# althonos/pyrodigal

Hardware: AMD Instinct MI355X
Metric: Mbp/sec gene-called (meta mode) (higher is better)
Workload: dtype f64; 1 GPU; 100000x20kbp_gc30-70_meta; contigs=100000, bases=2000000000, models=16, contigs_rank0=100000, sub_batch_contigs=6250, contexts_per_gpu=4, genes_all_ranks=2908995, steps_issued=a join of the contexts and a gather per step

## Files before the change

### pyrodigal_amd/csrc/finder.hip

```cpp
#include "pga_internal.h"
#include "pipeline.h"
#include "dpw_core.h"
#include "dev_common.h"
#include "find_plan.h"

#include <math.h>
#include <stdio.h>
#include <stdlib.h>
#include <string.h>

#include <algorithm>
#include <atomic>
#include <chrono>
#include <condition_variable>
#include <functional>
#include <limits>
#include <map>
#include <memory>
#include <mutex>
#include <new>
#include <thread>
#include <type_traits>
#include <unordered_map>

// ... 1004 lines not shown
    HT(c, hipMalloc((void**)&f->d_model_gc, sizeof(double) * nm));
    HT(c, hipMalloc((void**)&f->d_model_grp, sizeof(int32_t) * nm));
    HT(c, hipMemcpy(f->d_model_gc, mgc.data(), sizeof(double) * nm, hipMemcpyHostToDevice));
    HT(c, hipMemcpy(f->d_model_grp, f->model_group.data(), sizeof(int32_t) * nm, hipMemcpyHostToDevice));
    {
        const int ng = (int)f->group_tt.size();
        std::vector<int32_t> rank(nm, 0), count(ng, 0);
        for (int m = 0; m < nm; m++) rank[m] = count[f->model_group[m]]++;
        size_t total_il = 0;
        for (int g = 0; g < ng; g++) { f->gil_stride.push_back((count[g] + 1) & ~1); f->gil_off.push_back(total_il); total_il += (size_t)4096 * f->gil_stride[g]; }
        std::vector<double> il(total_il + 8, 0.0);
        for (int m = 0; m < nm; m++) {
            const int g = f->model_group[m];
            for (int h = 0; h < 4096; h++) il[f->gil_off[g] + (size_t)h * f->gil_stride[g] + rank[m]] = c->models[m].gene_dc[h];
        }
        HT(c, hipMalloc((void**)&f->d_gil, sizeof(double) * il.size()));
        HT(c, hipMalloc((void**)&f->d_model_rank, sizeof(int32_t) * nm));
        HT(c, hipMemcpy(f->d_gil, il.data(), sizeof(double) * il.size(), hipMemcpyHostToDevice));
        HT(c, hipMemcpy(f->d_model_rank, rank.data(), sizeof(int32_t) * nm, hipMemcpyHostToDevice));
        f->model_rank = rank;
    }
    return PGA_OK;
}

struct pga_batch {
    pga_ctx* ctx;
    int32_t n;
    int64_t total;
    std::vector<ContigDesc> ct;
    char* d_seq;
    size_t d_seq_cap = 0;
    TileDesc* d_tiles;
    int32_t* d_tile0;
    int32_t n_tiles;
    int mask_case = 0;
    std::vector<int32_t> reg_off;
    std::vector<MaskRun> regions;
    MaskRun* d_regions = nullptr;
    std::vector<uint8_t> circular;
    std::vector<int32_t> sets;
};

static void batch_tiles(const pga_batch* b, std::vector<TileDesc>& tiles, std::vector<int32_t>& tile0) {
    const int TS = pga_extract_tile_size();
    tile0.resize((size_t)b->n + 1);
    for (int i = 0; i < b->n; i++) {
        tile0[i] = (int32_t)tiles.size();
        const int64_t L = b->ct[i].len;
        if (L >= 3) for (int64_t s0 = 0; s0 < L; s0 += TS) tiles.push_back(TileDesc{i, (int32_t)s0});
    }
    tile0[b->n] = (int32_t)tiles.size();
}
static size_t batch_tiles_bytes(const std::vector<TileDesc>& tiles, const std::vector<int32_t>& tile0) {
    return sizeof(TileDesc) * tiles.size() + sizeof(int32_t) * tile0.size() + 64 + 256;
}
static hipError_t batch_upload_tiles(pga_batch* b, char* at, const std::vector<TileDesc>& tiles, const std::vector<int32_t>& tile0, hipStream_t st) {
    b->n_tiles = (int32_t)tiles.size();
    const size_t tb = sizeof(TileDesc) * tiles.size(), zb = sizeof(int32_t) * tile0.size();
    b->d_tiles = (TileDesc*)(((uintptr_t)at + 255) & ~(uintptr_t)255);
    b->d_tile0 = (int32_t*)((char*)b->d_tiles + tb);
    hipError_t e = hipSuccess;
    if (tb) e = hipMemcpyAsync(b->d_tiles, tiles.data(), tb, hipMemcpyHostToDevice, st);
    if (e == hipSuccess) e = hipMemcpyAsync(b->d_tile0, tile0.data(), zb, hipMemcpyHostToDevice, st);
    return e;
}

extern "C" int pga_dp_start_order(int32_t n_chains, const int32_t* nodes_per_chain, int32_t* order) {
    if (n_chains < 0 || (n_chains > 0 && (!nodes_per_chain || !order))) return PGA_EINVAL;
    int maxb = 0;
    for (int k = 0; k < n_chains; k++) maxb = std::max(maxb, std::max(nodes_per_chain[k], 0) >> 6);
    std::vector<int32_t> first((size_t)maxb + 2, 0);
    for (int k = 0; k < n_chains; k++) first[(size_t)(maxb - (std::max(nodes_per_chain[k], 0) >> 6)) + 1]++;
    for (int b = 0; b <= maxb; b++) first[(size_t)b + 1] += first[(size_t)b];
    for (int k = 0; k < n_chains; k++) order[(size_t)first[(size_t)(maxb - (std::max(nodes_per_chain[k], 0) >> 6))]++] = k;
    return PGA_OK;
}

extern "C" int64_t pga_dp_xcd_order(int32_t n_chains, const int32_t* order, const int32_t* nodes_per_chain, const int32_t* key_of_chain, int32_t n_keys,
                                    int32_t* out, int64_t out_cap) {
    if (n_chains < 0 || n_keys < 0 || (n_chains > 0 && (!order || !nodes_per_chain || !key_of_chain || !out))) return -(int64_t)PGA_EINVAL;
    std::vector<int32_t> queue[8];
    int64_t load[8] = {0, 0, 0, 0, 0, 0, 0, 0};
    std::vector<int8_t> xcd_of((size_t)n_keys, (int8_t)-1);
    for (int p = 0; p < n_chains; p++) {
        const int c = order[p];
        if (c < 0 || c >= n_chains || key_of_chain[c] < 0 || key_of_chain[c] >= n_keys) return -(int64_t)PGA_EINVAL;
        int8_t& x = xcd_of[(size_t)key_of_chain[c]];
        if (x < 0) { int best = 0; for (int q = 1; q < 8; q++) if (load[q] < load[best]) best = q; x = (int8_t)best; }
        queue[x].push_back(c);
        load[x] += std::max(nodes_per_chain[c], 0);
    }
    size_t longest = 0;
    for (int q = 0; q < 8; q++) longest = std::max(longest, queue[q].size());
// ... 420 lines not shown
    if (kn.fault_contig_len_set) {
        const long fl = kn.fault_contig_len;
        for (int i = 0; i < NC; i++) if ((long)batch->ct[i].len == fl) { c->err = "pga_find_genes: fault injected by PGA_FAULT_CONTIG_LEN"; return PGA_EDEVICE; }
    }
    if (use_sets) {
        NS = pga_plan::dense_set_ids(batch->sets.data(), NC, set_of);
        c->set_model.assign((size_t)NC, -1);
        c->set_score.assign((size_t)NC, std::numeric_limits<double>::quiet_NaN());
        c->model_scores.assign((size_t)NC * (size_t)NM, std::numeric_limits<double>::quiet_NaN());
        c->model_scores_nm = NM;
    }
    R = new (std::nothrow) ResultOwner();
    if (!R) return PGA_ENOMEM;
    R->contigs.assign(NC, pga_contig_result{-1, 0, 0, 0, 0, 0.0, 0.0});
    R->mask_off.assign(NC + 1, 0);
    R->has_masks = P.mask || mask_union;
    memset(&R->pub, 0, sizeof R->pub);
    R->pub.n_contigs = NC;
    total = batch->total;
    return PGA_OK;
}

int FindCall::run_sequence_and_masks() {
    const char* d_seq = batch->d_seq;
    DEVSET(d_dig, uint8_t, "d_dig", total + 16);
    DEVSET(d_ct, ContigDesc, "d_ct", NC + 1);
    const size_t xa_cnt = 4, xa_cbase = xa_cnt + 2 * (size_t)NC, xa_sbase = xa_cbase + (size_t)NG * (NC + 1), xa_en = xa_sbase + (size_t)NG * (NC + 1);
    xa_words = xa_en + ((size_t)NG * NC + 3) / 4 + 1;
    DEVSET(d_xa, int32_t, "d_extract_info", xa_words);
    PINSET(h_xa, int32_t, "h_extract_info", xa_words);
    d_cnt = d_xa + xa_cnt; h_cnt = h_xa + xa_cnt;
    const int64_t gc_blocks = pga_gc_blocks(total);
    DEVSET(d_p16, int32_t, "d_gc_p16", total / 16 + 2);
    DEVBUF(d_gc_bsum, int32_t, "d_gc_bsum", gc_blocks + 1);
    DEVBUF(d_gc_boff, int32_t, "d_gc_boff", gc_blocks + 1);
    d_cbase = d_xa + xa_cbase; h_cbase = h_xa + xa_cbase;
    DEVSET(d_tile_first, int32_t, "d_tile_first", (size_t)6 * batch->n_tiles);
    DEVSET(d_tile_last, int32_t, "d_tile_last", (size_t)6 * batch->n_tiles);
    DEVSET(d_tile.count, int32_t, "d_tile_count", (size_t)NG * (batch->n_tiles + 1));
    DEVSET(d_tile.off, int32_t, "d_tile_off", (size_t)NG * (batch->n_tiles + 1));
    DEVSET(d_tile.scount, int32_t, "d_tile_scount", (size_t)NG * (batch->n_tiles + 1));
    DEVSET(d_tile.soff, int32_t, "d_tile_soff", (size_t)NG * (batch->n_tiles + 1));
    d_sbase = d_xa + xa_sbase; h_sbase = h_xa + xa_sbase;
    d_enabled = (uint8_t*)(d_xa + xa_en); h_enabled = (uint8_t*)(h_xa + xa_en);

    for (int g = 0; g < NG; g++) {
        GBUF(df, uint8_t, total + 16)
        GBUF(c16, int32_t, (size_t)batch->n_tiles * 192 + 2)
        ga[g].tile0 = batch->d_tile0;
        ga[g].ndx = nullptr; ga[g].stop_val = nullptr; ga[g].type = nullptr; ga[g].strand = nullptr; ga[g].edge0 = nullptr; ga[g].gc_cont = nullptr;
    }

    HT(c, hipEventRecord(f->e_start, st));
    HT(c, hipMemcpyAsync(d_ct, batch->ct.data(), sizeof(ContigDesc) * (NC + 1), hipMemcpyHostToDevice, st));
    HT(c, hipMemsetAsync(d_xa, 0, sizeof(int32_t) * xa_cbase, st));
    pga_launch_digitize(d_seq, d_dig, total, d_ct, NC, d_cnt, d_cnt + NC, st);
    pga_launch_gc_prefix(d_dig, total, d_gc_bsum, d_gc_boff, d_p16, st);
    if (mask_union) {
        const int64_t per_source = total / std::max(1, P.min_mask) + NC + 1;
        const int64_t most = std::min<int64_t>((P.mask ? per_source : 0) + (batch->mask_case ? per_source : 0) + (int64_t)batch->regions.size(),
                                               total / 2 + NC + 1);
        const int cap = (int)std::min<int64_t>(most, (int64_t)1 << 28);
        DEVBUF(d_bits, uint32_t, "d_mask_bits", 2 * pga_mask_words(total) + 2);
        DEVBUF(d_mcounts, int32_t, "d_mask_counts", 4 * (pga_mask_waves(total) + 1));
        DEVBUF(d_moff, int32_t, "d_mask_off", NC + 2);
        DEVBUF(d_miv, int2, "d_mask_iv", cap + 1);
        PINBUF(h_moff_, int32_t, "h_mask_off", NC + 2);
        pga_launch_mask_union(d_dig, d_seq, total, d_ct, NC, batch->d_tiles, batch->n_tiles, P.mask, batch->mask_case, P.min_mask, batch->d_regions,
                              (int)batch->regions.size(), d_bits, d_mcounts, d_moff, d_miv, cap, st);
        HT(c, hipMemcpyAsync(h_moff_, d_moff, sizeof(int32_t) * (NC + 1), hipMemcpyDeviceToHost, st));
        h_moff = h_moff_; d_union_iv = d_miv;
        masks = MaskList{d_moff, d_miv};
    } else if (P.mask) {
        const int cap = (int)std::min<int64_t>(total / std::max(1, P.min_mask) + NC + 1, (int64_t)1 << 28);
        DEVBUF(d_runs, MaskRun, "d_mask_runs", cap + 1);
        DEVBUF(d_nruns, int32_t, "d_mask_count", 4);
        DEVBUF(d_moff, int32_t, "d_mask_off", NC + 2);
        DEVBUF(d_miv, int2, "d_mask_iv", cap + 1);
        pga_launch_find_masks(d_dig, d_ct, NC, batch->d_tiles, batch->n_tiles, P.min_mask, d_runs, d_nruns, cap, st);
        int32_t nruns = 0;
        HT(c, hipMemcpyAsync(&nruns, d_nruns, 4, hipMemcpyDeviceToHost, st));
        HT(c, hipStreamSynchronize(st));
        nruns = std::min(nruns, cap);
        std::vector<MaskRun> runs((size_t)nruns);
        if (nruns > 0) HT(c, hipMemcpy(runs.data(), d_runs, sizeof(MaskRun) * nruns, hipMemcpyDeviceToHost));
        std::sort(runs.begin(), runs.end(), [](const MaskRun& a, const MaskRun& b) { return a.contig != b.contig ? a.contig < b.contig : a.begin < b.begin; });
        std::vector<int32_t> moff(NC + 1, 0);
        std::vector<int2> miv((size_t)nruns + 1);
        for (int k = 0; k < nruns; k++) { moff[runs[k].contig + 1]++; miv[k] = make_int2(runs[k].begin, runs[k].end); }
        for (int i = 0; i < NC; i++) moff[i + 1] += moff[i];
// ... 1091 lines not shown
```

### pyrodigal_amd/csrc/pipeline.h

```cpp
#pragma once
#include "pga_internal.h"

#define PGA_STAGE_SLACK 8
struct TileDesc {
    int32_t contig;
    int32_t start;
};

struct GroupArrays {
    uint8_t* df;
    int32_t* c16; const int32_t* tile0 = nullptr;
    int32_t* st_ndx; int32_t* st_sv;
    uint8_t* st_info;
    int32_t st_half = 0; int32_t* st_overflow = nullptr;
    int32_t* stop_list;
    int32_t* start_list = nullptr;
    uint32_t* ovl_topo;
    int32_t* srank = nullptr;
    int32_t* ndx; int32_t* stop_val; uint8_t* type; int8_t* strand; uint8_t* edge0; float* gc_cont;
    int32_t* contig_of = nullptr;
};

struct ChainArrays {
    double* cscore; double* sscore; double* rscore; double* uscore; double* tscore; double* mot_score;
    double* cscore_raw;
    int32_t* star_ptr;
    int32_t* mot_ndx;
    uint8_t* rbs;
    uint8_t* edge;
    uint8_t* mot_len; uint8_t* mot_spacer; uint8_t* mot_spacendx;
    double* cs_sink = nullptr;
};

struct ModelScoreConst {
    double lfac_min, lfac_max;
    double lfac_tab[1001];
};

struct MaskList {
    const int32_t* off;
    const int2* iv;
};
struct MaskRun { int32_t contig, begin, end, _pad; };

struct ScoreParams {
    int32_t closed, is_meta, max_overlap, n_models;
    double* cs_out;
    uint8_t* conv_flag;
    unsigned long long* prof = nullptr;
    int32_t models_per_pass = 512;
    int32_t lean_stops = 0;
};

void pga_launch_digitize(const char* d_seq, uint8_t* d_dig, int64_t total, const ContigDesc* d_ct, int n_contigs,
                         int32_t* d_gc, int32_t* d_unk, hipStream_t st);
int64_t pga_gc_blocks(int64_t total);
void pga_launch_gc_prefix(const uint8_t* d_dig, int64_t total, int32_t* d_block_sum, int32_t* d_block_off, int32_t* d_p16, hipStream_t st);
void pga_launch_extract(const uint8_t* d_dig, int64_t total, const ContigDesc* d_ct, int n_contigs, int tt,
                        const pga_params& p, const GroupArrays& ga, const TileDesc* d_tiles, int n_tiles, const int32_t* d_tile0,
                        int32_t* d_tile_first, int32_t* d_tile_last, int32_t* d_tile_count, int32_t* d_tile_off, int32_t* d_cbase,
                        int32_t* d_tile_scount, int32_t* d_tile_soff, int32_t* d_sbase ,
                        MaskList masks, hipStream_t st,
                        const uint8_t* d_enabled = nullptr ,
                        int ex_c = 4 ,
                        int ex_pool = 128 );
void pga_launch_place(const ContigDesc* d_ct, const TileDesc* d_tiles, int n_tiles, const int32_t* d_tile_off, const int32_t* d_tile_soff,
                      const GroupArrays& ga, hipStream_t st);
int32_t pga_mm_tiles(const ChainDesc* h_chains, int n_chains, const int32_t* h_cbase, const int32_t* h_sbase, int n_models, int tile, std::vector<int64_t>& scratch);
size_t pga_mm_scratch_bytes(int n_models, int n_chains);
constexpr size_t PGA_SS_REC_BYTES = 32, PGA_SS_MMCHAIN_BYTES = 32, PGA_SS_MMTILE_BYTES = 16;
void pga_launch_group_enable(const ContigDesc* d_ct, int n_contigs, const int32_t* d_gc_count, const double* d_model_gc,
                             const int32_t* d_model_group, int n_models, int n_groups, uint8_t* d_enabled, hipStream_t st);
void pga_launch_group_enable_sets(const ContigDesc* d_ct, int n_contigs, const int32_t* d_gc_count, const int32_t* d_set_of, int32_t* d_pool,
                                  const double* d_model_gc, const int32_t* d_model_group, int n_models, int n_groups, uint8_t* d_enabled,
                                  hipStream_t st);
void pga_launch_find_masks(const uint8_t* d_dig, const ContigDesc* d_ct, int n_contigs, const TileDesc* d_tiles, int n_tiles, int min_mask,
                           MaskRun* d_runs, int32_t* d_count, int cap, hipStream_t st);
int64_t pga_mask_words(int64_t total);
int64_t pga_mask_waves(int64_t total);
void pga_launch_mask_union(const uint8_t* d_dig, const char* d_seq, int64_t total, const ContigDesc* d_ct, int n_contigs, const TileDesc* d_tiles,
                           int n_tiles, int unknown_runs, int lower_case_runs, int min_mask, const MaskRun* d_regions, int n_regions,
                           uint32_t* d_bits, int32_t* d_counts, int32_t* d_moff, int2* d_miv, int cap, hipStream_t st);
int pga_extract_tile_size();
void pga_launch_orf_gc(const ContigDesc* d_ct, int n_contigs, const uint8_t* d_dig, const int32_t* d_p16, const GroupArrays& ga,
                       int n_nodes_total, const int32_t* d_node_contig_base, hipStream_t st);
struct ScoreGroup {
    const ChainDesc* d_chains = nullptr; int n_chains = 0; int64_t node_begin = 0, total = 0;
    const ChainDesc* d_all_chains = nullptr; const int2* d_contig_chains = nullptr;
    const int32_t* d_node_contig_base = nullptr; int n_contigs = 0; int group_nodes = 0;
    const uint8_t* d_dig = nullptr; const ContigDesc* d_ct = nullptr; const GroupArrays* ga = nullptr; const ChainArrays* ca = nullptr;
// ... 38 lines not shown
```

### pyrodigal_amd/csrc/pipeline.hip

```cpp

#include "pga_internal.h"
#include "pipeline.h"
#include <atomic>
#include "dev_common.h"
#include "dpw_core.h"

namespace {

enum { NA = 0, NG = 1, NC = 2, NT = 3, NN = 6 };

__device__ __forceinline__ int find_contig(const ContigDesc* __restrict__ ct, int n, int64_t g) {
    int lo = 0, hi = n - 1;
    while (lo < hi) { int mid = (lo + hi + 1) >> 1; if (ct[mid].base <= g) lo = mid; else hi = mid - 1; }
    return lo;
}

__device__ __forceinline__ int block_contig(const ContigDesc* __restrict__ ct, int n, int64_t block_first, int64_t g, int* s_slot) {
    int c = block_search_le([&](const int k) { return ct[k].base; }, n, block_first, s_slot);
    while (c + 1 < n && ct[c + 1].base <= g) c++;
    return c;
}
__device__ __forceinline__ int block_chain(const ChainDesc* __restrict__ ch, int n, int64_t block_first, int64_t g, int* s_slot) {
    int c = block_search_le([&](const int k) { return ch[k].off; }, n, block_first, s_slot);
    while (c + 1 < n && ch[c + 1].off <= g) c++;
    return c;
}

__device__ __forceinline__ double readlane_f64_pl(double v, int lane) {
    const int lo = __builtin_amdgcn_readlane(__double2loint(v), lane);
    const int hi = __builtin_amdgcn_readlane(__double2hiint(v), lane);
    return __hiloint2double(hi, lo);
}

__device__ __forceinline__ int sbase(const uint8_t* __restrict__ d, int L, int i, int strand) {
    return strand == 1 ? d[i] : (d[L - 1 - i] ^ 3);
}
__device__ __forceinline__ int comp2(int d) { return d <= 3 ? (d ^ 3) : NN; }
__device__ __forceinline__ int is_gc_n(int d) { return d != NA && d != NT; }

__host__ __device__ __forceinline__ bool codon_is_stop(int x0, int x1, int x2, int tt) {
    if (x0 != NT) {
        if (tt == 2) return x0 == NA && x1 == NG && (x2 == NA || x2 == NG);
        return false;
    }
    const unsigned long long taa = (1ULL<<1)|(1ULL<<2)|(1ULL<<3)|(1ULL<<4)|(1ULL<<5)|(1ULL<<9)|(1ULL<<10)|(1ULL<<11)|(1ULL<<12)|(1ULL<<13)
                                 | (1ULL<<15)|(1ULL<<16)|(1ULL<<21)|(1ULL<<22)|(1ULL<<23)|(1ULL<<24)|(1ULL<<25)|(1ULL<<26)|(1ULL<<32);
    const unsigned long long tag = (1ULL<<1)|(1ULL<<2)|(1ULL<<3)|(1ULL<<4)|(1ULL<<5)|(1ULL<<9)|(1ULL<<10)|(1ULL<<11)|(1ULL<<12)|(1ULL<<13)
                                 | (1ULL<<14)|(1ULL<<21)|(1ULL<<23)|(1ULL<<24)|(1ULL<<25)|(1ULL<<26)|(1ULL<<33);
    const unsigned long long tga = (1ULL<<1)|(1ULL<<6)|(1ULL<<11)|(1ULL<<12)|(1ULL<<15)|(1ULL<<16)|(1ULL<<22)|(1ULL<<23)|(1ULL<<26)
                                 | (1ULL<<29)|(1ULL<<30)|(1ULL<<32);
    if (x1 == NA && x2 == NG) return (tag >> tt) & 1;
    if (x1 == NG && x2 == NA) return (tga >> tt) & 1;
    if (x1 == NA && x2 == NA) return (taa >> tt) & 1;
    if (tt == 22) return x1 == NC && x2 == NA;
// ... 4 lines not shown
    if (x1 != NT || x2 != NG) return false;
    if (x0 == NA) return true;
    if (tt == 6 || tt == 10 || tt == 14 || tt == 15 || tt == 16 || tt == 2) return false;
    if (x0 == NG) return !(tt == 1 || tt == 3 || tt == 12 || tt == 2);
    if (x0 == NT) return !(tt < 4 || tt == 9 || (tt >= 21 && tt < 25));
    return false;
}
__device__ __forceinline__ bool is_stop_at(const uint8_t* __restrict__ d, int L, int i, int strand, int tt) {
    return codon_is_stop(sbase(d, L, i, strand), sbase(d, L, i + 1, strand), sbase(d, L, i + 2, strand), tt);
}

__device__ __forceinline__ int digit_of(int ch, int& gc, int& unk) {
    switch (ch) {
        case 'A': case 'a': return NA;
        case 'T': case 't': return NT;
        case 'G': case 'g': gc++; return NG;
        case 'C': case 'c': gc++; return NC;
        default: unk++; return NN;
    }
}

__device__ __forceinline__ unsigned digits4(const unsigned w, int& gc, int& unk) {
    const unsigned u = w & 0xdfdfdfdfu;
    auto eq = [](const unsigned v) {
        return (~(((v & 0x7f7f7f7fu) + 0x7f7f7f7fu) | v | 0x7f7f7f7fu)) >> 7;
    };
    const unsigned a = eq(u ^ 0x41414141u), g = eq(u ^ 0x47474747u), c = eq(u ^ 0x43434343u), t = eq(u ^ 0x54545454u);
    const unsigned n = ~(a | g | c | t) & 0x01010101u;
    gc += __popc(g | c); unk += __popc(n);
    return g | (c << 1) | t | (t << 1) | (n << 1) | (n << 2);
}

constexpr int DG_BLOCK = 16384;
__global__ void __launch_bounds__(256)
k_digitize(const char* __restrict__ seq, uint8_t* __restrict__ dig, int64_t total,
           const ContigDesc* __restrict__ ct, int n_contigs, int32_t* __restrict__ gc_count, int32_t* __restrict__ unk_count) {
    __shared__ int s_c0;
    const int64_t blk0 = (int64_t)blockIdx.x * DG_BLOCK;
    int c = block_contig(ct, n_contigs, blk0, blk0, &s_c0);
    uint4 v[4];
#pragma unroll
    for (int q = 0; q < 4; q++) {
        const int64_t g0 = blk0 + q * 4096 + (int64_t)threadIdx.x * 16;
        v[q] = g0 + 16 <= total ? *reinterpret_cast<const uint4*>(seq + g0) : make_uint4(0, 0, 0, 0);
    }
    int acc_c = -1, acc_gc = 0, acc_unk = 0;
#pragma unroll
    for (int q = 0; q < 4; q++) {
        const int64_t g0 = blk0 + q * 4096 + (int64_t)threadIdx.x * 16;
        const bool in = g0 < total;
        if (in) while (c + 1 < n_contigs && ct[c + 1].base <= g0) c++;
        int gc = 0, unk = 0;
        bool one_contig = true;
        if (in) {
            const int64_t next = ct[c + 1 <= n_contigs ? c + 1 : n_contigs].base;
            if (g0 + 16 <= total && g0 + 16 <= next) {
                const uint4 o = make_uint4(digits4(v[q].x, gc, unk), digits4(v[q].y, gc, unk), digits4(v[q].z, gc, unk), digits4(v[q].w, gc, unk));
                *reinterpret_cast<uint4*>(dig + g0) = o;
            } else {
                one_contig = false;
                int cc = c;
                for (int k = 0; k < 16 && g0 + k < total; k++) {
                    const int64_t g = g0 + k;
                    while (cc + 1 < n_contigs && ct[cc + 1].base <= g) cc++;
                    int a = 0, u = 0;
                    dig[g] = (uint8_t)digit_of(seq[g], a, u);
                    if (a) atomicAdd(&gc_count[cc], 1);
                    if (u) atomicAdd(&unk_count[cc], 1);
                }
            }
        }
        const int c0 = __builtin_amdgcn_readfirstlane(c);
        const bool uniform = __all(!in || (one_contig && c == c0));
        if (uniform) {
            int a = in ? gc : 0, u = in ? unk : 0;
#pragma unroll
            for (int m = 32; m >= 1; m >>= 1) { a += __shfl_xor(a, m, 64); u += __shfl_xor(u, m, 64); }
            if (acc_c != c0) {
                if ((threadIdx.x & 63) == 0 && acc_c >= 0) { if (acc_gc) atomicAdd(&gc_count[acc_c], acc_gc); if (acc_unk) atomicAdd(&unk_count[acc_c], acc_unk); }
                acc_c = c0; acc_gc = 0; acc_unk = 0;
            }
            acc_gc += a; acc_unk += u;
        } else if (in && one_contig) {
            if (gc) atomicAdd(&gc_count[c], gc);
            if (unk) atomicAdd(&unk_count[c], unk);
        }
    }
    __shared__ int s_c[4], s_g[4], s_u[4];
    const int wv = threadIdx.x >> 6;
    if ((threadIdx.x & 63) == 0) { s_c[wv] = acc_c; s_g[wv] = acc_gc; s_u[wv] = acc_unk; }
    __syncthreads();
    if (threadIdx.x == 0) {
#pragma unroll
        for (int w = 0; w < 4; w++) {
            if (s_c[w] < 0) continue;
            int g = s_g[w], u = s_u[w];
#pragma unroll
            for (int v = w + 1; v < 4; v++) if (s_c[v] == s_c[w]) { g += s_g[v]; u += s_u[v]; s_c[v] = -1; }
            if (g) atomicAdd(&gc_count[s_c[w]], g);
            if (u) atomicAdd(&unk_count[s_c[w]], u);
        }
    }
}

constexpr int EX_TILE = 3072;
constexpr int EX_PER_THREAD = 12;
constexpr int EX_NONE_HI = 0x7fffffff;

__device__ __forceinline__ unsigned pack4(const unsigned w, const bool comp) {
    unsigned c = w & 0x03030303u;
    if (comp) { const unsigned nm = (w >> 2) & 0x01010101u; c = (c ^ 0x03030303u) ^ (nm | (nm << 1)); }
    return (c | (c >> 6) | (c >> 12) | (c >> 18)) & 0xffu;
}
__device__ __forceinline__ unsigned long long pack16(const uint4 v, const bool comp) {
    return (unsigned long long)(pack4(v.x, comp) | (pack4(v.y, comp) << 8) | (pack4(v.z, comp) << 16) | (pack4(v.w, comp) << 24));
}
__device__ __forceinline__ unsigned long long pairrev64(unsigned long long x) {
    x = __brevll(x);
    return ((x & 0x5555555555555555ull) << 1) | ((x >> 1) & 0x5555555555555555ull);
}

struct TileGeom {
    int L, a, len;
// ... 482 lines not shown
            const int ndx = ga.st_ndx[s0 + j], info = ga.st_info[s0 + j];
            k = off + j;
            ga.ndx[k] = ndx; ga.stop_val[k] = ga.st_sv[s0 + j]; ga.type[k] = info & 3; ga.strand[k] = (info >> 3) & 1 ? -1 : 1; ga.edge0[k] = (info >> 2) & 1;
            ga.contig_of[k] = td.contig;
            const int g_hi = (ndx - td.start) >> 4, g_lo = j == 0 ? 0 : ((ga.st_ndx[s0 + j - 1] - td.start) >> 4) + 1;
            for (int g = g_lo; g <= g_hi; g++) c16[g] = k;
            if (j == cnt - 1) for (int g = g_hi + 1; g < n_groups; g++) c16[g] = off + cnt;
            is_stop = (info & 3) == PGA_T_STOP;
        }
        const unsigned long long bal = __ballot(is_stop);
        if (lane == 0) s_w[wv] = __popcll(bal);
        __syncthreads();
        const int stops_before = srun + (wv ? s_w[0] : 0) + __popcll(bal & ((1ull << lane) - 1ull));
        if (is_stop) ga.stop_list[stops_before] = k;
        else if (j < cnt && ga.start_list != nullptr) ga.start_list[start0 + j - (stops_before - tile_soff[blockIdx.x])] = k;
        srun += s_w[0] + s_w[1];
        __syncthreads();
    }
}

__device__ __forceinline__ int gcn16(const uint4 v, const int nbytes ) {
    const unsigned w[4] = {v.x, v.y, v.z, v.w};
    int n = 0;
#pragma unroll
    for (int q = 0; q < 4; q++) {
        unsigned b = (w[q] ^ (w[q] >> 1)) & 0x01010101u;
        const int keep = nbytes - 4 * q;
        if (keep <= 0) b = 0; else if (keep < 4) b &= (1u << (8 * keep)) - 1u;
        n += __popc(b);
    }
    return n;
}
__global__ void __launch_bounds__(256)
k_gcp_blocks(const uint8_t* __restrict__ dig, int64_t total, int32_t* __restrict__ block_sum) {
    __shared__ int s_w[4];
    const int64_t g0 = (int64_t)blockIdx.x * 4096 + (int64_t)threadIdx.x * 16;
    int n = 0;
    if (g0 < total) n = gcn16(*reinterpret_cast<const uint4*>(dig + g0), (int)min((int64_t)16, total - g0));
#pragma unroll
    for (int m = 32; m >= 1; m >>= 1) n += __shfl_xor(n, m, 64);
    if ((threadIdx.x & 63) == 0) s_w[threadIdx.x >> 6] = n;
    __syncthreads();
    if (threadIdx.x == 0) block_sum[blockIdx.x] = s_w[0] + s_w[1] + s_w[2] + s_w[3];
}
__global__ void __launch_bounds__(256)
k_gcp_final(const uint8_t* __restrict__ dig, int64_t total, const int32_t* __restrict__ block_off, int32_t* __restrict__ p16) {
    __shared__ int s_w[4];
    const int64_t g0 = (int64_t)blockIdx.x * 4096 + (int64_t)threadIdx.x * 16;
    int n = 0;
    if (g0 < total) n = gcn16(*reinterpret_cast<const uint4*>(dig + g0), (int)min((int64_t)16, total - g0));
    int inc = n;
    const int lane = threadIdx.x & 63, w = threadIdx.x >> 6;
#pragma unroll
    for (int off = 1; off < 64; off <<= 1) { const int v = __shfl_up(inc, off, 64); if (lane >= off) inc += v; }
    if (lane == 63) s_w[w] = inc;
    __syncthreads();
    int run = block_off[blockIdx.x] + inc - n;
    for (int k = 0; k < w; k++) run += s_w[k];
    if (g0 <= total) p16[g0 >> 4] = run;
}
__device__ __forceinline__ int gc_prefix(const uint8_t* __restrict__ dig, const int32_t* __restrict__ p16, const int64_t x) {
    const int r = (int)(x & 15);
    int n = p16[x >> 4];
    if (r) n += gcn16(*reinterpret_cast<const uint4*>(dig + (x - r)), r);
    return n;
}

__global__ void __launch_bounds__(256)
k_orf_gc(const ContigDesc* __restrict__ ct, int n_contigs, const uint8_t* __restrict__ dig, const int32_t* __restrict__ p16, GroupArrays ga,
         int n_nodes_total, const int32_t* __restrict__ node_contig_base ) {
    const int i = blockIdx.x * blockDim.x + threadIdx.x;
    if (i >= n_nodes_total) return;
    if (ga.type[i] == PGA_T_STOP) { ga.gc_cont[i] = 0.f; return; }
    const int lo = ga.contig_of[i];
    const int L = ct[lo].len;
    const int64_t base = ct[lo].base;
    auto P = [&](const int x) { return gc_prefix(dig, p16, base + x); };
    const int ndx = ga.ndx[i], sv = ga.stop_val[i];
    int cnt;
    if (ga.strand[i] == 1) {
        cnt = P(sv + 3) - P(ndx);
    } else {
        const int hi2 = min(ndx + 2, L - 1);
        cnt = (P(sv + 1) - P(sv - 2)) + (hi2 >= sv + 3 ? P(hi2 + 1) - P(sv + 3) : 0);
    }
    const double gsize = abs(sv - ndx) + 3.0;
    ga.gc_cont[i] = (float)((double)cnt / gsize);
}

__device__ __forceinline__ int hexamer(const uint8_t* __restrict__ d, int pos, int strand) {
    int v = 0;
    if (strand == 1) { for (int j = 0; j < 6; j++) v |= (d[pos + j] & 3) << (2 * j); }
    else             { for (int j = 0; j < 6; j++) v |= (comp2(d[pos - j] & 7) & 3) << (2 * j); }
    return v;
}

constexpr int CS_MODELS = 4;
constexpr int CS_LONG = 192;
constexpr int CSQ_SERIAL_MAX = 256;

struct OrfCtx {
    const uint8_t* d;
    const int32_t* c16;
    int tbase, p, q, L, strand, step, ncod;
    int kstop;
    int2 cc;
    __device__ __forceinline__ bool node_at(const int j) const { return (d[j] >> (strand == 1 ? 4 : 5)) & 1; }
    __device__ __forceinline__ int node_index(const int j) const {
        const int r = j & 15;
        uint4 v; __builtin_memcpy(&v, d + (j - r), 16);
        const unsigned w[4] = {v.x, v.y, v.z, v.w};
        int n = c16[j >> 4] - tbase;
#pragma unroll
        for (int q = 0; q < 4; q++) {
            const int keep = r - 4 * q;
            unsigned m = w[q] & 0x30303030u;
            if (keep <= 0) m = 0; else if (keep < 4) m &= (1u << (8 * keep)) - 1u;
// ... 1788 lines not shown
    const OvlChain C{ga.ndx + tb, ga.stop_val + tb, ga.type + tb, ga.strand + tb, ca.cscore + ch.off, ca.sscore + ch.off, ca.rscore + ch.off,
                     ca.uscore + ch.off, ch.n, css != nullptr ? css + ch.off : nullptr};
    overlapping_starts_ahead(C, i, my, !rev, mc, maxov, sp, K, edge0 != 1 ? neighbours : 0x80000000u, ext != nullptr ? topo_q2 + tb : nullptr);
    ca.star_ptr[3 * g] = sp[0]; ca.star_ptr[3 * g + 1] = sp[1]; ca.star_ptr[3 * g + 2] = sp[2];
    if (ext != nullptr) {
        DpwExt e;
        e.vm = 0;
#pragma unroll
        for (int k = 0; k < 3; k++) {
            e.x[k] = 0.0; e.dlo[k] = INT_MAX; e.dhi[k] = INT_MIN; e.cq[k] = DPW_NONE;
            if (sp[k] < 0) continue;
            e.vm |= 1 << k;
            e.x[k] = K.v[k];
            if (rev && e.x[k] > 0.0) {
                const int n3n = K.nd[k], n3s = K.sv[k];
                int hi = n3s + DPW_MAX_OPP_OVLP - 5;
                const int h2 = (n3n + n3s - 6) >> 1;
                if (h2 < hi) hi = h2;
                if (my - 4 < hi) hi = my - 4;
                e.dlo[k] = n3s - 5; e.dhi[k] = hi;
            }
            if (rev) e.cq[k] = K.q2[k];
        }
        ext[p] = e;
    }
}

}

static inline unsigned nblocks(int64_t n, int t) { return (unsigned)((n + t - 1) / t); }

int64_t pga_gc_blocks(int64_t total) { return (total + 1 + 4095) / 4096; }

void pga_launch_digitize(const char* d_seq, uint8_t* d_dig, int64_t total, const ContigDesc* d_ct, int n_contigs,
                         int32_t* d_gc, int32_t* d_unk, hipStream_t st) {
    if (total <= 0) return;
    hipLaunchKernelGGL(k_digitize, dim3(nblocks(total, DG_BLOCK)), dim3(256), 0, st, d_seq, d_dig, total, d_ct, n_contigs, d_gc, d_unk);
}

struct RunOfUnknown {
    static __device__ __forceinline__ bool is(const uint8_t b) { return b == NN; }
    static __device__ __forceinline__ bool all8(const uint64_t w) { return w == 0x0606060606060606ull; }
};
struct RunOfLowerCase {
    static __device__ __forceinline__ bool is(const uint8_t b) { return (unsigned)(b - 'a') < 26u; }
    static __device__ __forceinline__ bool all8(const uint64_t w) {
        const uint64_t H = 0x8080808080808080ull;
        if (w & H) return false;
        return ((w + 0x1f1f1f1f1f1f1f1full) & H) == H
            && ((w + 0x0505050505050505ull) & H) == 0;
    }
};

template <class Run, class Emit>
__device__ __forceinline__ void find_runs(const uint8_t* __restrict__ src, const ContigDesc* __restrict__ ct, const TileDesc* __restrict__ tiles,
                                          const int n_tiles, const int n_contigs, const int min_mask, Emit emit) {
    if ((int)blockIdx.x >= n_tiles) {
        const int c = ((int)blockIdx.x - n_tiles) * blockDim.x + threadIdx.x;
        if (c >= n_contigs) return;
        const ContigDesc cd = ct[c];
        if (cd.len < 1 || cd.len > 2) return;
        const uint8_t* __restrict__ d = src + cd.base;
        for (int i = 0; i < cd.len; i++) {
            if (!Run::is(d[i]) || (i > 0 && Run::is(d[i - 1]))) continue;
            int e = i + 1;
            while (e < cd.len && Run::is(d[e])) e++;
            if (e - i >= min_mask || e == cd.len) emit(c, i, e);
        }
        return;
    }
// ... 127 lines not shown
        S &= S - 1u;
        if (ks < cap) iv[ks].x = (int)(g - ct[find_contig(ct, n_contigs, g)].base);
        ks++;
    }
    while (E) {
        const int64_t g = w * 32 + __builtin_ctz(E);
        E &= E - 1u;
        if (ke < cap) iv[ke].y = (int)(g + 1 - ct[find_contig(ct, n_contigs, g)].base);
        ke++;
    }
}

int64_t pga_mask_words(int64_t total) { return (total + 32) / 32; }
int64_t pga_mask_waves(int64_t total) { return (pga_mask_words(total) + 63) / 64; }

void pga_launch_mask_union(const uint8_t* d_dig, const char* d_seq, int64_t total, const ContigDesc* d_ct, int n_contigs, const TileDesc* d_tiles,
                           int n_tiles, int unknown_runs, int lower_case_runs, int min_mask, const MaskRun* d_regions, int n_regions,
                           uint32_t* d_bits, int32_t* d_counts, int32_t* d_moff, int2* d_miv, int cap, hipStream_t st) {
    const int64_t nw = pga_mask_words(total), nwv = pga_mask_waves(total);
    uint32_t* const d_cbits = d_bits + nw;
    int32_t* const cnt_s = d_counts; int32_t* const cnt_e = cnt_s + (nwv + 1); int32_t* const off_s = cnt_e + (nwv + 1); int32_t* const off_e = off_s + (nwv + 1);
    (void)hipMemsetAsync(d_bits, 0, sizeof(uint32_t) * 2 * (size_t)nw, st);
    const dim3 run_grid(n_tiles + (n_contigs + 255) / 256);
    if (unknown_runs) hipLaunchKernelGGL(k_mask_paint_runs<RunOfUnknown>, run_grid, dim3(256), 0, st, d_dig, d_ct, d_tiles, n_tiles, n_contigs, min_mask, d_bits);
    if (lower_case_runs) hipLaunchKernelGGL(k_mask_paint_runs<RunOfLowerCase>, run_grid, dim3(256), 0, st, (const uint8_t*)d_seq, d_ct, d_tiles, n_tiles, n_contigs, min_mask, d_bits);
    hipLaunchKernelGGL(k_mask_paint_regions, dim3((n_regions + 3) / 4 + (n_contigs + 255) / 256), dim3(256), 0, st, d_regions, n_regions, d_ct, n_contigs, d_bits, d_cbits);
    const int word_blocks = (int)((nw + 255) / 256);
    hipLaunchKernelGGL(k_mask_count, dim3(word_blocks), dim3(256), 0, st, (const uint32_t*)d_bits, (const uint32_t*)d_cbits, nw, cnt_s, cnt_e);
    hipLaunchKernelGGL(k_scan_counts, dim3(1), dim3(1024), 0, st, (const int32_t*)cnt_s, (int)nwv, off_s, (const int32_t*)cnt_e, off_e);
    hipLaunchKernelGGL(k_mask_place, dim3(word_blocks + (n_contigs + 1 + 255) / 256), dim3(256), 0, st, (const uint32_t*)d_bits, (const uint32_t*)d_cbits, nw, word_blocks,
                       (const int32_t*)off_s, (const int32_t*)off_e, d_ct, n_contigs, d_moff, d_miv, cap);
}

void pga_launch_gc_prefix(const uint8_t* d_dig, int64_t total, int32_t* d_block_sum, int32_t* d_block_off, int32_t* d_p16, hipStream_t st) {
    if (total <= 0) return;
    const int nb = (int)pga_gc_blocks(total);
    hipLaunchKernelGGL(k_gcp_blocks, dim3(nb), dim3(256), 0, st, d_dig, total, d_block_sum);
    hipLaunchKernelGGL(k_scan_counts, dim3(1), dim3(1024), 0, st, d_block_sum, nb, d_block_off, (const int32_t*)nullptr, (int32_t*)nullptr);
    hipLaunchKernelGGL(k_gcp_final, dim3(nb), dim3(256), 0, st, d_dig, total, d_block_off, d_p16);
}

void pga_launch_extract(const uint8_t* d_dig, int64_t total, const ContigDesc* d_ct, int n_contigs, int tt,
                        const pga_params& p, const GroupArrays& ga, const TileDesc* d_tiles, int n_tiles, const int32_t* d_tile0,
                        int32_t* d_tile_first, int32_t* d_tile_last, int32_t* d_tile_count, int32_t* d_tile_off, int32_t* d_cbase,
                        int32_t* d_tile_scount, int32_t* d_tile_soff, int32_t* d_sbase, MaskList masks, hipStream_t st, const uint8_t* d_enabled,
                        int ex_c, int ex_pool) {
    if (n_tiles > 0) {
        ExParams P{tt, p.closed, p.min_gene, p.min_edge_gene, 0ull, 0ull, std::min(ex_c, EX_C), std::max(0, std::min(ex_pool, EX_POOL))};
        for (int idx = 0; idx < 64; idx++) {
            const int b0 = idx & 3, b1 = (idx >> 2) & 3, b2 = (idx >> 4) & 3;
            if (codon_is_stop(b0, b1, b2, tt)) P.stop_codons |= 1ull << idx;
            if (codon_is_start(b0, b1, b2, tt)) P.start_codons |= 1ull << idx;
        }
        hipLaunchKernelGGL(k_tile_stops, dim3(n_tiles), dim3(64), 0, st, d_dig, total, d_ct, d_tiles, n_tiles, P.stop_codons, d_tile_first, d_tile_last, d_enabled);
        if (P.ex_c > 0)
            hipLaunchKernelGGL(k_extract_tile<true>, dim3(n_tiles), dim3(256), 0, st, d_dig, total, d_ct, d_tiles, n_tiles, d_tile_first, d_tile_last, P, ga, masks,
                               d_enabled, d_tile_count, d_tile_scount);
        else
            hipLaunchKernelGGL(k_extract_tile<false>, dim3(n_tiles), dim3(256), 0, st, d_dig, total, d_ct, d_tiles, n_tiles, d_tile_first, d_tile_last, P, ga, masks,
                               d_enabled, d_tile_count, d_tile_scount);
    }
    hipLaunchKernelGGL(k_scan_counts, dim3(1), dim3(1024), 0, st, d_tile_count, n_tiles, d_tile_off, (const int32_t*)d_tile_scount, d_tile_soff);
    hipLaunchKernelGGL(k_contig_node_base, dim3((n_contigs + 1 + 255) / 256), dim3(256), 0, st, d_tile0, n_contigs, d_tile_off, d_cbase);
    hipLaunchKernelGGL(k_contig_node_base, dim3((n_contigs + 1 + 255) / 256), dim3(256), 0, st, d_tile0, n_contigs, d_tile_soff, d_sbase);
}

void pga_launch_place(const ContigDesc* d_ct, const TileDesc* d_tiles, int n_tiles, const int32_t* d_tile_off, const int32_t* d_tile_soff,
                      const GroupArrays& ga, hipStream_t st) {
    if (n_tiles <= 0) return;
    hipLaunchKernelGGL(k_place_nodes, dim3(n_tiles), dim3(128), 0, st, d_ct, d_tiles, d_tile_off, d_tile_soff, ga);
}

int pga_extract_tile_size() { return EX_TILE; }

// ... 54 lines not shown
__global__ void __launch_bounds__(256)
k_set_pool(const ContigDesc* __restrict__ ct, int n_contigs, const int32_t* __restrict__ gc_count, const int32_t* __restrict__ set_of,
           int32_t* __restrict__ pool) {
    const int i = blockIdx.x * blockDim.x + threadIdx.x;
    if (i >= n_contigs) return;
    const int s = set_of[i];
    if (s < 0 || s >= n_contigs) return;
    atomicAdd(pool + 2 * (size_t)s, gc_count[i]);
    atomicAdd(pool + 2 * (size_t)s + 1, (int32_t)ct[i].len);
}
__global__ void __launch_bounds__(256)
k_group_enable_sets(int n_contigs, const int32_t* __restrict__ set_of, const int32_t* __restrict__ pool, const double* __restrict__ model_gc,
                    const int32_t* __restrict__ model_group, int n_models, int n_groups, uint8_t* __restrict__ enabled ) {
    const int i = blockIdx.x * blockDim.x + threadIdx.x;
    if (i >= n_contigs) return;
    const int s = set_of[i];
    const bool ok = s >= 0 && s < n_contigs;
    const int L = ok ? pool[2 * (size_t)s + 1] : 0;
    const double gc = L > 0 ? (double)pool[2 * (size_t)s] / (double)L : 0.0;
    const double low = fmin(0.65, 0.88495 * gc - 0.0102337), high = fmax(0.35, 0.86596 * gc + 0.1131991);
    unsigned need = 0;
    for (int m = 0; m < n_models; m++) if (!(model_gc[m] < low || model_gc[m] > high)) need |= 1u << model_group[m];
    for (int g = 0; g < n_groups; g++) enabled[(size_t)g * n_contigs + i] = (need >> g) & 1;
}
void pga_launch_group_enable_sets(const ContigDesc* d_ct, int n_contigs, const int32_t* d_gc_count, const int32_t* d_set_of, int32_t* d_pool,
                                  const double* d_model_gc, const int32_t* d_model_group, int n_models, int n_groups, uint8_t* d_enabled,
                                  hipStream_t st) {
    if (n_contigs <= 0) return;
    (void)hipMemsetAsync(d_pool, 0, sizeof(int32_t) * 2 * (size_t)n_contigs, st);
    hipLaunchKernelGGL(k_set_pool, dim3(nblocks(n_contigs, 256)), dim3(256), 0, st, d_ct, n_contigs, d_gc_count, d_set_of, d_pool);
    hipLaunchKernelGGL(k_group_enable_sets, dim3(nblocks(n_contigs, 256)), dim3(256), 0, st, n_contigs, d_set_of, d_pool, d_model_gc, d_model_group,
                       n_models, n_groups, d_enabled);
}



void pga_launch_orf_gc(const ContigDesc* d_ct, int n_contigs, const uint8_t* d_dig, const int32_t* d_p16, const GroupArrays& ga,
                       int n_nodes_total, const int32_t* d_node_contig_base, hipStream_t st) {
    if (n_nodes_total <= 0) return;
    hipLaunchKernelGGL(k_orf_gc, dim3(nblocks(n_nodes_total, 256)), dim3(256), 0, st, d_ct, n_contigs, d_dig, d_p16, ga,
                       n_nodes_total, d_node_contig_base);
}

void pga_launch_sd_lut(unsigned* d_lut, hipStream_t st) {
    hipLaunchKernelGGL(k_sd_lut, dim3((PGA_SD_LUT + 255) / 256), dim3(256), 0, st, d_lut);
}

int32_t pga_mm_tiles(const ChainDesc* h_chains, int n_chains, const int32_t* h_cbase, const int32_t* h_sbase, int n_models, int tile, std::vector<int64_t>& items) {
    items.assign((size_t)n_models, 0);
    for (int k = 0; k < n_chains; k++) {
        const int c = h_chains[k].contig;
        items[(size_t)h_chains[k].model] += (h_cbase[c + 1] - h_cbase[c]) - (h_sbase[c + 1] - h_sbase[c]);
    }
    int64_t tiles = 0;
    for (int m = 0; m < n_models; m++) tiles += (items[(size_t)m] + tile - 1) / tile;
    return (int32_t)tiles;
}
size_t pga_mm_scratch_bytes(int n_models, int n_chains) {
    return sizeof(unsigned long long) * SS_CNT_STRIDE * (size_t)n_models + sizeof(int32_t) * (((size_t)3 * n_models + 1) & ~(size_t)1) + sizeof(int2) * (size_t)n_chains + 64;
}

enum ProfileKind { PROF_CS, PROF_SS };
static unsigned long long* profile_begin(const ProfileKind kind, hipStream_t st) {
    static std::atomic<unsigned long long*> prof_of[2][64];
    int dev = 0;
    (void)hipGetDevice(&dev);
    dev &= 63;
// ... 102 lines not shown
```

Measured before the change: 21550 Mbp/s.

## Fuse GC prefix-sum block counting into digitize kernel with precomputed block contigs

The digitize kernel now also computes per-16-base local GC prefix values and per-4096-base block sums with wave scans. This replaces the separate block-sum and final kernels that re-read the digitized sequence, leaving only a block scan and a cheap add kernel. Block-to-contig lookup is precomputed on the host and uploaded with the tiles, which removes the in-kernel binary search. Non-uniform waves now merge atomics per contig run, and the ORF GC count uses one fewer prefix lookup. The cost is an extra uint16 buffer and a more complex digitize kernel with more shuffles.

```diff
diff --git a/pyrodigal_amd/csrc/finder.hip b/pyrodigal_amd/csrc/finder.hip
--- a/pyrodigal_amd/csrc/finder.hip
+++ b/pyrodigal_amd/csrc/finder.hip
@@ -1060,6 +1060,7 @@
     size_t d_seq_cap = 0;
     TileDesc* d_tiles;
     int32_t* d_tile0;
+    int32_t* d_blk_contig = nullptr;
     int32_t n_tiles;
     int mask_case = 0;
     std::vector<int32_t> reg_off;
@@ -1071,13 +1072,19 @@
 
 static void batch_tiles(const pga_batch* b, std::vector<TileDesc>& tiles, std::vector<int32_t>& tile0) {
     const int TS = pga_extract_tile_size();
-    tile0.resize((size_t)b->n + 1);
+    const int64_t total = b->ct[b->n].base, blocks = pga_gc_blocks(total);
+    tile0.resize((size_t)b->n + 1 + (size_t)blocks);
     for (int i = 0; i < b->n; i++) {
         tile0[i] = (int32_t)tiles.size();
         const int64_t L = b->ct[i].len;
         if (L >= 3) for (int64_t s0 = 0; s0 < L; s0 += TS) tiles.push_back(TileDesc{i, (int32_t)s0});
     }
     tile0[b->n] = (int32_t)tiles.size();
+    int c = 0;
+    for (int64_t j = 0; j < blocks; j++) {
+        while (c + 1 < b->n && b->ct[c + 1].base <= j * 4096) c++;
+        tile0[(size_t)b->n + 1 + (size_t)j] = c;
+    }
 }
 static size_t batch_tiles_bytes(const std::vector<TileDesc>& tiles, const std::vector<int32_t>& tile0) {
     return sizeof(TileDesc) * tiles.size() + sizeof(int32_t) * tile0.size() + 64 + 256;
@@ -1087,6 +1094,7 @@
     const size_t tb = sizeof(TileDesc) * tiles.size(), zb = sizeof(int32_t) * tile0.size();
     b->d_tiles = (TileDesc*)(((uintptr_t)at + 255) & ~(uintptr_t)255);
     b->d_tile0 = (int32_t*)((char*)b->d_tiles + tb);
+    b->d_blk_contig = b->d_tile0 + b->n + 1;
     hipError_t e = hipSuccess;
     if (tb) e = hipMemcpyAsync(b->d_tiles, tiles.data(), tb, hipMemcpyHostToDevice, st);
     if (e == hipSuccess) e = hipMemcpyAsync(b->d_tile0, tile0.data(), zb, hipMemcpyHostToDevice, st);
@@ -1573,6 +1581,7 @@
     d_cnt = d_xa + xa_cnt; h_cnt = h_xa + xa_cnt;
     const int64_t gc_blocks = pga_gc_blocks(total);
     DEVSET(d_p16, int32_t, "d_gc_p16", total / 16 + 2);
+    DEVBUF(d_gc_l16, uint16_t, "d_gc_l16", total / 16 + 2);
     DEVBUF(d_gc_bsum, int32_t, "d_gc_bsum", gc_blocks + 1);
     DEVBUF(d_gc_boff, int32_t, "d_gc_boff", gc_blocks + 1);
     d_cbase = d_xa + xa_cbase; h_cbase = h_xa + xa_cbase;
@@ -1595,8 +1604,7 @@
     HT(c, hipEventRecord(f->e_start, st));
     HT(c, hipMemcpyAsync(d_ct, batch->ct.data(), sizeof(ContigDesc) * (NC + 1), hipMemcpyHostToDevice, st));
     HT(c, hipMemsetAsync(d_xa, 0, sizeof(int32_t) * xa_cbase, st));
-    pga_launch_digitize(d_seq, d_dig, total, d_ct, NC, d_cnt, d_cnt + NC, st);
-    pga_launch_gc_prefix(d_dig, total, d_gc_bsum, d_gc_boff, d_p16, st);
+    pga_launch_digitize(d_seq, d_dig, total, d_ct, NC, batch->d_blk_contig, d_cnt, d_cnt + NC, d_gc_l16, d_gc_bsum, d_gc_boff, d_p16, st);
     if (mask_union) {
         const int64_t per_source = total / std::max(1, P.min_mask) + NC + 1;
         const int64_t most = std::min<int64_t>((P.mask ? per_source : 0) + (batch->mask_case ? per_source : 0) + (int64_t)batch->regions.size(),
diff --git a/pyrodigal_amd/csrc/pipeline.h b/pyrodigal_amd/csrc/pipeline.h
--- a/pyrodigal_amd/csrc/pipeline.h
+++ b/pyrodigal_amd/csrc/pipeline.h
@@ -52,10 +52,10 @@
     int32_t lean_stops = 0;
 };
 
-void pga_launch_digitize(const char* d_seq, uint8_t* d_dig, int64_t total, const ContigDesc* d_ct, int n_contigs,
-                         int32_t* d_gc, int32_t* d_unk, hipStream_t st);
 int64_t pga_gc_blocks(int64_t total);
-void pga_launch_gc_prefix(const uint8_t* d_dig, int64_t total, int32_t* d_block_sum, int32_t* d_block_off, int32_t* d_p16, hipStream_t st);
+void pga_launch_digitize(const char* d_seq, uint8_t* d_dig, int64_t total, const ContigDesc* d_ct, int n_contigs, const int32_t* d_blk_contig,
+                         int32_t* d_gc, int32_t* d_unk, uint16_t* d_l16, int32_t* d_block_sum, int32_t* d_block_off, int32_t* d_p16,
+                         hipStream_t st);
 void pga_launch_extract(const uint8_t* d_dig, int64_t total, const ContigDesc* d_ct, int n_contigs, int tt,
                         const pga_params& p, const GroupArrays& ga, const TileDesc* d_tiles, int n_tiles, const int32_t* d_tile0,
                         int32_t* d_tile_first, int32_t* d_tile_last, int32_t* d_tile_count, int32_t* d_tile_off, int32_t* d_cbase,
diff --git a/pyrodigal_amd/csrc/pipeline.hip b/pyrodigal_amd/csrc/pipeline.hip
--- a/pyrodigal_amd/csrc/pipeline.hip
+++ b/pyrodigal_amd/csrc/pipeline.hip
@@ -15,11 +15,6 @@
     return lo;
 }
 
-__device__ __forceinline__ int block_contig(const ContigDesc* __restrict__ ct, int n, int64_t block_first, int64_t g, int* s_slot) {
-    int c = block_search_le([&](const int k) { return ct[k].base; }, n, block_first, s_slot);
-    while (c + 1 < n && ct[c + 1].base <= g) c++;
-    return c;
-}
 __device__ __forceinline__ int block_chain(const ChainDesc* __restrict__ ch, int n, int64_t block_first, int64_t g, int* s_slot) {
     int c = block_search_le([&](const int k) { return ch[k].off; }, n, block_first, s_slot);
     while (c + 1 < n && ch[c + 1].off <= g) c++;
@@ -90,28 +85,33 @@
 }
 
 constexpr int DG_BLOCK = 16384;
+constexpr int GCP_BLOCK = 4096;
 __global__ void __launch_bounds__(256)
 k_digitize(const char* __restrict__ seq, uint8_t* __restrict__ dig, int64_t total,
-           const ContigDesc* __restrict__ ct, int n_contigs, int32_t* __restrict__ gc_count, int32_t* __restrict__ unk_count) {
-    __shared__ int s_c0;
-    const int64_t blk0 = (int64_t)blockIdx.x * DG_BLOCK;
-    int c = block_contig(ct, n_contigs, blk0, blk0, &s_c0);
+           const ContigDesc* __restrict__ ct, int n_contigs, const int32_t* __restrict__ blk_contig,
+           int32_t* __restrict__ gc_count, int32_t* __restrict__ unk_count, uint16_t* __restrict__ l16, int32_t* __restrict__ block_sum) {
+    const int lane = threadIdx.x & 63, wv = threadIdx.x >> 6;
+    const int pb = blockIdx.x * (DG_BLOCK / GCP_BLOCK) + wv;
+    const int64_t wv0 = (int64_t)pb * GCP_BLOCK;
     uint4 v[4];
 #pragma unroll
     for (int q = 0; q < 4; q++) {
-        const int64_t g0 = blk0 + q * 4096 + (int64_t)threadIdx.x * 16;
+        const int64_t g0 = wv0 + q * 1024 + lane * 16;
         v[q] = g0 + 16 <= total ? *reinterpret_cast<const uint4*>(seq + g0) : make_uint4(0, 0, 0, 0);
     }
+    int c = 0;
+    int64_t next = total;
+    if (wv0 <= total) { c = blk_contig[pb]; next = ct[c + 1].base; }
     int acc_c = -1, acc_gc = 0, acc_unk = 0;
+    int before = 0;
 #pragma unroll
     for (int q = 0; q < 4; q++) {
-        const int64_t g0 = blk0 + q * 4096 + (int64_t)threadIdx.x * 16;
+        const int64_t g0 = wv0 + q * 1024 + lane * 16;
         const bool in = g0 < total;
-        if (in) while (c + 1 < n_contigs && ct[c + 1].base <= g0) c++;
+        if (in) while (c + 1 < n_contigs && next <= g0) { c++; next = ct[c + 1].base; }
         int gc = 0, unk = 0;
         bool one_contig = true;
         if (in) {
-            const int64_t next = ct[c + 1 <= n_contigs ? c + 1 : n_contigs].base;
             if (g0 + 16 <= total && g0 + 16 <= next) {
                 const uint4 o = make_uint4(digits4(v[q].x, gc, unk), digits4(v[q].y, gc, unk), digits4(v[q].z, gc, unk), digits4(v[q].w, gc, unk));
                 *reinterpret_cast<uint4*>(dig + g0) = o;
@@ -125,28 +125,40 @@
                     dig[g] = (uint8_t)digit_of(seq[g], a, u);
                     if (a) atomicAdd(&gc_count[cc], 1);
                     if (u) atomicAdd(&unk_count[cc], 1);
+                    gc += a; unk += u;
                 }
             }
         }
+        const int mine = gc | (unk << 16);
+        int inc = mine;
+#pragma unroll
+        for (int o = 1; o < 64; o <<= 1) { const int x = __shfl_up(inc, o, 64); if (lane >= o) inc += x; }
+        const int ex = inc - mine, all = __builtin_amdgcn_readlane(inc, 63);
+        if (g0 <= total) l16[g0 >> 4] = (uint16_t)(before + (ex & 0xffff) + (ex >> 16));
+        before += (all & 0xffff) + (all >> 16);
         const int c0 = __builtin_amdgcn_readfirstlane(c);
         const bool uniform = __all(!in || (one_contig && c == c0));
         if (uniform) {
-            int a = in ? gc : 0, u = in ? unk : 0;
-#pragma unroll
-            for (int m = 32; m >= 1; m >>= 1) { a += __shfl_xor(a, m, 64); u += __shfl_xor(u, m, 64); }
             if (acc_c != c0) {
-                if ((threadIdx.x & 63) == 0 && acc_c >= 0) { if (acc_gc) atomicAdd(&gc_count[acc_c], acc_gc); if (acc_unk) atomicAdd(&unk_count[acc_c], acc_unk); }
+                if (lane == 0 && acc_c >= 0) { if (acc_gc) atomicAdd(&gc_count[acc_c], acc_gc); if (acc_unk) atomicAdd(&unk_count[acc_c], acc_unk); }
                 acc_c = c0; acc_gc = 0; acc_unk = 0;
             }
-            acc_gc += a; acc_unk += u;
-        } else if (in && one_contig) {
-            if (gc) atomicAdd(&gc_count[c], gc);
-            if (unk) atomicAdd(&unk_count[c], unk);
-        }
-    }
+            acc_gc += all & 0xffff; acc_unk += all >> 16;
+        } else {
+            unsigned long long todo = __ballot(in && one_contig);
+            while (todo) {
+                const int first = __ffsll(todo) - 1;
+                const int cr = __builtin_amdgcn_readlane(c, first);
+                const unsigned long long run = __ballot(in && one_contig && c == cr);
+                const int sum = __builtin_amdgcn_readlane(inc, 63 - __clzll(run)) - __builtin_amdgcn_readlane(ex, first);
+                if (lane == 0) { if (sum & 0xffff) atomicAdd(&gc_count[cr], sum & 0xffff); if (sum >> 16) atomicAdd(&unk_count[cr], sum >> 16); }
+                todo &= ~run;
+            }
+        }
+    }
+    if (lane == 0 && wv0 <= total) block_sum[pb] = before;
     __shared__ int s_c[4], s_g[4], s_u[4];
-    const int wv = threadIdx.x >> 6;
-    if ((threadIdx.x & 63) == 0) { s_c[wv] = acc_c; s_g[wv] = acc_gc; s_u[wv] = acc_unk; }
+    if (lane == 0) { s_c[wv] = acc_c; s_g[wv] = acc_gc; s_u[wv] = acc_unk; }
     __syncthreads();
     if (threadIdx.x == 0) {
 #pragma unroll
@@ -695,32 +707,9 @@
     return n;
 }
 __global__ void __launch_bounds__(256)
-k_gcp_blocks(const uint8_t* __restrict__ dig, int64_t total, int32_t* __restrict__ block_sum) {
-    __shared__ int s_w[4];
-    const int64_t g0 = (int64_t)blockIdx.x * 4096 + (int64_t)threadIdx.x * 16;
-    int n = 0;
-    if (g0 < total) n = gcn16(*reinterpret_cast<const uint4*>(dig + g0), (int)min((int64_t)16, total - g0));
-#pragma unroll
-    for (int m = 32; m >= 1; m >>= 1) n += __shfl_xor(n, m, 64);
-    if ((threadIdx.x & 63) == 0) s_w[threadIdx.x >> 6] = n;
-    __syncthreads();
-    if (threadIdx.x == 0) block_sum[blockIdx.x] = s_w[0] + s_w[1] + s_w[2] + s_w[3];
-}
-__global__ void __launch_bounds__(256)
-k_gcp_final(const uint8_t* __restrict__ dig, int64_t total, const int32_t* __restrict__ block_off, int32_t* __restrict__ p16) {
-    __shared__ int s_w[4];
-    const int64_t g0 = (int64_t)blockIdx.x * 4096 + (int64_t)threadIdx.x * 16;
-    int n = 0;
-    if (g0 < total) n = gcn16(*reinterpret_cast<const uint4*>(dig + g0), (int)min((int64_t)16, total - g0));
-    int inc = n;
-    const int lane = threadIdx.x & 63, w = threadIdx.x >> 6;
-#pragma unroll
-    for (int off = 1; off < 64; off <<= 1) { const int v = __shfl_up(inc, off, 64); if (lane >= off) inc += v; }
-    if (lane == 63) s_w[w] = inc;
-    __syncthreads();
-    int run = block_off[blockIdx.x] + inc - n;
-    for (int k = 0; k < w; k++) run += s_w[k];
-    if (g0 <= total) p16[g0 >> 4] = run;
+k_gcp_p16(const uint16_t* __restrict__ l16, const int32_t* __restrict__ block_off, int64_t n16, int32_t* __restrict__ p16) {
+    const int64_t i = (int64_t)blockIdx.x * 256 + threadIdx.x;
+    if (i < n16) p16[i] = block_off[i >> 8] + l16[i];
 }
 __device__ __forceinline__ int gc_prefix(const uint8_t* __restrict__ dig, const int32_t* __restrict__ p16, const int64_t x) {
     const int r = (int)(x & 15);
@@ -745,7 +734,8 @@
         cnt = P(sv + 3) - P(ndx);
     } else {
         const int hi2 = min(ndx + 2, L - 1);
-        cnt = (P(sv + 1) - P(sv - 2)) + (hi2 >= sv + 3 ? P(hi2 + 1) - P(sv + 3) : 0);
+        if (hi2 >= sv + 3) cnt = P(hi2 + 1) - P(sv - 2) - is_gc_n(dig[base + sv + 1]) - is_gc_n(dig[base + sv + 2]);
+        else cnt = P(sv + 1) - P(sv - 2);
     }
     const double gsize = abs(sv - ndx) + 3.0;
     ga.gc_cont[i] = (float)((double)cnt / gsize);
@@ -2600,10 +2590,16 @@
 
 int64_t pga_gc_blocks(int64_t total) { return (total + 1 + 4095) / 4096; }
 
-void pga_launch_digitize(const char* d_seq, uint8_t* d_dig, int64_t total, const ContigDesc* d_ct, int n_contigs,
-                         int32_t* d_gc, int32_t* d_unk, hipStream_t st) {
+void pga_launch_digitize(const char* d_seq, uint8_t* d_dig, int64_t total, const ContigDesc* d_ct, int n_contigs, const int32_t* d_blk_contig,
+                         int32_t* d_gc, int32_t* d_unk, uint16_t* d_l16, int32_t* d_block_sum, int32_t* d_block_off, int32_t* d_p16,
+                         hipStream_t st) {
     if (total <= 0) return;
-    hipLaunchKernelGGL(k_digitize, dim3(nblocks(total, DG_BLOCK)), dim3(256), 0, st, d_seq, d_dig, total, d_ct, n_contigs, d_gc, d_unk);
+    hipLaunchKernelGGL(k_digitize, dim3(nblocks(total + 1, DG_BLOCK)), dim3(256), 0, st, d_seq, d_dig, total, d_ct, n_contigs, d_blk_contig,
+                       d_gc, d_unk, d_l16, d_block_sum);
+    const int nb = (int)pga_gc_blocks(total);
+    hipLaunchKernelGGL(k_scan_counts, dim3(1), dim3(1024), 0, st, (const int32_t*)d_block_sum, nb, d_block_off, (const int32_t*)nullptr, (int32_t*)nullptr);
+    const int64_t n16 = total / 16 + 1;
+    hipLaunchKernelGGL(k_gcp_p16, dim3(nblocks(n16, 256)), dim3(256), 0, st, (const uint16_t*)d_l16, (const int32_t*)d_block_off, n16, d_p16);
 }
 
 struct RunOfUnknown {
@@ -2797,14 +2793,6 @@
                        (const int32_t*)off_s, (const int32_t*)off_e, d_ct, n_contigs, d_moff, d_miv, cap);
 }
 
-void pga_launch_gc_prefix(const uint8_t* d_dig, int64_t total, int32_t* d_block_sum, int32_t* d_block_off, int32_t* d_p16, hipStream_t st) {
-    if (total <= 0) return;
-    const int nb = (int)pga_gc_blocks(total);
-    hipLaunchKernelGGL(k_gcp_blocks, dim3(nb), dim3(256), 0, st, d_dig, total, d_block_sum);
-    hipLaunchKernelGGL(k_scan_counts, dim3(1), dim3(1024), 0, st, d_block_sum, nb, d_block_off, (const int32_t*)nullptr, (int32_t*)nullptr);
-    hipLaunchKernelGGL(k_gcp_final, dim3(nb), dim3(256), 0, st, d_dig, total, d_block_off, d_p16);
-}
-
 void pga_launch_extract(const uint8_t* d_dig, int64_t total, const ContigDesc* d_ct, int n_contigs, int tt,
                         const pga_params& p, const GroupArrays& ga, const TileDesc* d_tiles, int n_tiles, const int32_t* d_tile0,
                         int32_t* d_tile_first, int32_t* d_tile_last, int32_t* d_tile_count, int32_t* d_tile_off, int32_t* d_cbase,
@@ -2925,7 +2913,6 @@
     hipLaunchKernelGGL(k_group_enable_sets, dim3(nblocks(n_contigs, 256)), dim3(256), 0, st, n_contigs, d_set_of, d_pool, d_model_gc, d_model_group,
                        n_models, n_groups, d_enabled);
 }
-
 
 
 void pga_launch_orf_gc(const ContigDesc* d_ct, int n_contigs, const uint8_t* d_dig, const int32_t* d_p16, const GroupArrays& ga,
```

Measured after the change: 22050 Mbp/s, median of 4. +2.3%, better.
